# martenlienen/generative-turbulence

Measured on AMD Instinct MI355X. Metric: U-Net fwd+bwd voxels/sec (DDPM training step, 192x64x48x4), higher is better.
Workload: dtype bf16

## Files before the change

### generative-turbulence_amd/csrc/tdx_resize.hip

```cpp
#include "tdx_common.h"
#include <stdlib.h>

struct AxisMap {
    int in, out;
    float scale;
};
__host__ __device__ inline AxisMap make_axis(int in, int out) {
    AxisMap a;
    a.in = in; a.out = out;
    a.scale = out > 1 ? (float)(in - 1) / (float)(out - 1) : 0.0f;
    return a;
}
__host__ __device__ __forceinline__ void axis_taps(const AxisMap& a, int o, int& i0, int& i1, float& w1) {
    const float src = a.scale * (float)o;
    i0 = min((int)src, a.in - 1);
    w1 = fminf(fmaxf(src - (float)i0, 0.0f), 1.0f);
    i1 = i0 + ((i0 + 1 < a.in) ? 1 : 0);
}

struct TileGrid {
    int nx, ny, nz;
    int sy, sz;
    int tx, ty, tz;
};
// ... 192 lines not shown
}
__host__ __device__ __forceinline__ void axis_span(const AxisMap& a, int i, int& first, int& cnt) {
    int lo, hi;
    axis_range(a, i, lo, hi);
    first = hi + 1;
    int last = lo - 1;
    for (int o = lo; o <= hi; ++o)
        if (axis_weight(a, o, i) != 0.f) {
            first = min(first, o);
            last = o;
        }
    cnt = last - first + 1;
    if (cnt < 0) cnt = 0;
}

template <typename T, int K>
__global__ void __launch_bounds__(256)
resize_bwd_kernel(const T* __restrict__ dy, const T* __restrict__ add, T* __restrict__ dx, AxisMap ax, AxisMap ay, AxisMap az,
                  int C, TileGrid tg) {
    __shared__ int s_first[3][RS_MAXT], s_cnt[3][RS_MAXT];
    __shared__ float s_w[3][RS_MAXT][RS_KMAX];
    int b, ix0, iy0, iz0;
    tile_origin(tg, b, ix0, iy0, iz0);
    if (threadIdx.x < 3 * RS_MAXT) {
        const int a = threadIdx.x / RS_MAXT, k = threadIdx.x % RS_MAXT;
        const AxisMap& m = a == 0 ? ax : (a == 1 ? ay : az);
        const int i = min((a == 0 ? ix0 : (a == 1 ? iy0 : iz0)) + k, m.in - 1);
        int f, c;
        axis_span(m, i, f, c);
        s_first[a][k] = f; s_cnt[a][k] = c;
        for (int j = 0; j < RS_KMAX; ++j) s_w[a][k][j] = j < c ? axis_weight(m, f + j, i) : 0.f;
    }
    __syncthreads();
    const int L = C >> 3;
    const int per_pass = 256 / L;
    const int lc = (int)threadIdx.x % L;
    const int nvox = tg.tx * tg.ty * tg.tz;
    if ((int)threadIdx.x >= per_pass * L) return;
    for (int slot = (int)threadIdx.x / L; slot < nvox; slot += per_pass) {
        const int kz = slot & (tg.tz - 1), ky = (slot >> tg.sz) & (tg.ty - 1), kx = slot >> (tg.sz + tg.sy);
        const int ix = ix0 + kx, iy = iy0 + ky, iz = iz0 + kz;
        if (ix >= ax.in || iy >= ay.in || iz >= az.in) continue;
        const int fx = s_first[0][kx], cx = s_cnt[0][kx], fy = s_first[1][ky], cy = s_cnt[1][ky], fz = s_first[2][kz];
        float wz[K];
        int oz[K];
#pragma unroll
        for (int k = 0; k < K; ++k) {
            oz[k] = min(fz + k, az.out - 1);
            wz[k] = s_w[2][kz][k];
        }
        const T* gb = dy + ((int64_t)b * ax.out * ay.out * az.out) * C + lc * 8;
        float acc[8];
#pragma unroll
        for (int j = 0; j < 8; ++j) acc[j] = 0.f;
        for (int a = 0; a < cx; ++a) {
            const float wx = s_w[0][kx][a];
            for (int bb = 0; bb < cy; ++bb) {
                const float wxy = wx * s_w[1][ky][bb];
                const T* row = gb + (((int64_t)(fx + a) * ay.out + (fy + bb)) * az.out) * C;
                Raw8<T> t[K];
#pragma unroll
                for (int k = 0; k < K; ++k) t[k].load(row + (int64_t)oz[k] * C);
                __builtin_amdgcn_sched_barrier(0);
#pragma unroll
                for (int k = 0; k < K; ++k) {
                    const float w = wxy * wz[k];
                    const Vec8<T> v = t[k].get();
#pragma unroll
                    for (int j = 0; j < 8; ++j) acc[j] += w * v.v[j];
                }
            }
        }
        const int64_t di = ((((int64_t)b * ax.in + ix) * ay.in + iy) * az.in + iz) * C + lc * 8;
        if (add != nullptr) {
            Vec8<T> a;
            a.load(add + di);
#pragma unroll
            for (int j = 0; j < 8; ++j) acc[j] += a.v[j];
        }
        Vec8<T> o;
#pragma unroll
        for (int j = 0; j < 8; ++j) o.v[j] = acc[j];
        o.store(dx + di);
    }
}

template <typename T>
__global__ void __launch_bounds__(256)
resize_bwd_generic_kernel(const T* __restrict__ dy, const T* __restrict__ add, T* __restrict__ dx, AxisMap ax, AxisMap ay,
                          AxisMap az, int C, int64_t total) {
    const int L = C >> 3;
    int64_t i = (int64_t)blockIdx.x * blockDim.x + threadIdx.x;
    if (i >= total) return;
    const int lc = (int)(i % L);
    int64_t v = i / L;
    const int iz = (int)(v % az.in); v /= az.in;
    const int iy = (int)(v % ay.in); v /= ay.in;
    const int ix = (int)(v % ax.in);
    const int b = (int)(v / ax.in);
    int x0, x1, y0, y1, z0, z1;
    axis_range(ax, ix, x0, x1);
    axis_range(ay, iy, y0, y1);
    axis_range(az, iz, z0, z1);
    const T* gb = dy + ((int64_t)b * ax.out * ay.out * az.out) * C + lc * 8;
    float acc[8];
#pragma unroll
    for (int j = 0; j < 8; ++j) acc[j] = 0.f;
    for (int ox = x0; ox <= x1; ++ox) {
        const float wx = axis_weight(ax, ox, ix);
        if (wx == 0.f) continue;
        for (int oy = y0; oy <= y1; ++oy) {
            const float wxy = wx * axis_weight(ay, oy, iy);
            if (wxy == 0.f) continue;
            const T* row = gb + (((int64_t)ox * ay.out + oy) * az.out) * C;
            for (int oz = z0; oz <= z1; ++oz) {
                const float w = wxy * axis_weight(az, oz, iz);
                if (w == 0.f) continue;
                Vec8<T> t;
                t.load(row + (int64_t)oz * C);
#pragma unroll
                for (int j = 0; j < 8; ++j) acc[j] += w * t.v[j];
            }
        }
    }
    const int64_t di = ((((int64_t)b * ax.in + ix) * ay.in + iy) * az.in + iz) * C + lc * 8;
    if (add != nullptr) {
        Vec8<T> a;
        a.load(add + di);
#pragma unroll
        for (int j = 0; j < 8; ++j) acc[j] += a.v[j];
    }
    Vec8<T> o;
#pragma unroll
    for (int j = 0; j < 8; ++j) o.v[j] = acc[j];
    o.store(dx + di);
}

static int resize_args_ok(int B, int Xi, int Yi, int Zi, int Xo, int Yo, int Zo, int C) {
    return B > 0 && Xi > 0 && Yi > 0 && Zi > 0 && Xo > 0 && Yo > 0 && Zo > 0 && C > 0;
}
static TileGrid make_tiles(int X, int Y, int Z, int C, int64_t samples = 0) {
    const int L = C >> 3;
    int vox = 256;
    while (vox > 8 && vox * L > 8 * 256) vox >>= 1;
    const int one_pass = 256 / L > 8 ? 256 / L : 8;
    while (samples > 0 && vox > one_pass && samples * X * Y * Z / vox < 1024) vox >>= 1;
    TileGrid t;
    t.tz = 8; t.ty = 8; t.tx = 4;
    while (t.tx * t.ty * t.tz > vox && t.tx > 1) t.tx >>= 1;
    while (t.tx * t.ty * t.tz > vox && t.ty > 1) t.ty >>= 1;
    while (t.tx * t.ty * t.tz > vox && t.tz > 1) t.tz >>= 1;
    t.sy = 0; while ((1 << t.sy) < t.ty) ++t.sy;
    t.sz = 0; while ((1 << t.sz) < t.tz) ++t.sz;
    t.nx = ceil_div(X, t.tx); t.ny = ceil_div(Y, t.ty); t.nz = ceil_div(Z, t.tz);
    return t;
}
extern "C" int tdx_resize_fwd(const void* x, void* y, int B, int Xi, int Yi, int Zi, int Xo, int Yo, int Zo, int C,
                              int dtype, void* stream) {
    TDX_CHECK_ARG(x && y && resize_args_ok(B, Xi, Yi, Zi, Xo, Yo, Zo, C));
    if (C % 8 || C / 8 > 256) return TDX_ESHAPE;
    const TileGrid tg = make_tiles(Xo, Yo, Zo, C, B);
    const int64_t blocks = (int64_t)B * tg.nx * tg.ny * tg.nz;
    const AxisMap mx = make_axis(Xi, Xo), my = make_axis(Yi, Yo), mz = make_axis(Zi, Zo);
    if (C <= 64 && !((tg.tx | tg.ty | tg.tz) & 1) && Xo > Xi && Yo > Yi && Zo > Zi && pair_window_ok(mx) &&
        pair_window_ok(my) && pair_window_ok(mz)) {
        TDX_DISPATCH_DTYPE(dtype, hipLaunchKernelGGL((resize_up_pairs_kernel<T>), dim3((unsigned)blocks), dim3(256), 0,
                                                      as_stream(stream), (const T*)x, (T*)y, mx, my, mz, C, tg));
        return tdx_launch_status();
    }
    TDX_DISPATCH_DTYPE(dtype, hipLaunchKernelGGL((resize_fwd_kernel<T>), dim3((unsigned)blocks), dim3(256), 0,
                                                  as_stream(stream), (const T*)x, (T*)y, make_axis(Xi, Xo),
                                                  make_axis(Yi, Yo), make_axis(Zi, Zo), C, tg));
    return tdx_launch_status();
}

static int axis_max_span(const AxisMap& a) {
    int m = 0;
    for (int i = 0; i < a.in; ++i) {
        int f, c;
        axis_span(a, i, f, c);
        m = c > m ? c : m;
    }
    return m;
}

extern "C" int tdx_resize_bwd(const void* dy, const void* add, void* dx, int B, int Xi, int Yi, int Zi, int Xo, int Yo, int Zo, int C,
                              int dtype, void* stream) {
    TDX_CHECK_ARG(dy && dx && resize_args_ok(B, Xi, Yi, Zi, Xo, Yo, Zo, C));
    if (C % 8 || C / 8 > 256) return TDX_ESHAPE;
    const AxisMap ax = make_axis(Xi, Xo), ay = make_axis(Yi, Yo), az = make_axis(Zi, Zo);
    const int kx = axis_max_span(ax), ky = axis_max_span(ay), kz = axis_max_span(az);
    if (kx > RS_KMAX || ky > RS_KMAX || kz > RS_KMAX) {
        const int64_t total = (int64_t)B * Xi * Yi * Zi * (C / 8);
        TDX_DISPATCH_DTYPE(dtype, hipLaunchKernelGGL((resize_bwd_generic_kernel<T>), dim3(ceil_div(total, 256)), dim3(256), 0,
                                                      as_stream(stream), (const T*)dy, (const T*)add, (T*)dx, ax, ay, az, C, total));
        return tdx_launch_status();
    }
    const TileGrid tg = make_tiles(Xi, Yi, Zi, C, B);
    const dim3 grid((unsigned)((int64_t)B * tg.nx * tg.ny * tg.nz));
#define RS_BWD(KV)                                                                                                     \
    TDX_DISPATCH_DTYPE(dtype, hipLaunchKernelGGL((resize_bwd_kernel<T, KV>), grid, dim3(256), 0, as_stream(stream),     \
                                                  (const T*)dy, (const T*)add, (T*)dx, ax, ay, az, C, tg))
    if (kz <= 2) RS_BWD(2);
    else if (kz <= 4) RS_BWD(4);
    else if (kz <= 6) RS_BWD(6);
    else RS_BWD(RS_KMAX);
#undef RS_BWD
    return tdx_launch_status();
}
```

### generative-turbulence_amd/turbdiff_amd/_lib.py

```python

from __future__ import annotations

import ctypes as C
import os
import threading
from pathlib import Path

import torch

_HERE = Path(__file__).resolve().parent
LIB_PATH = Path(os.environ.get("TDX_LIB", _HERE / "libtdx_hip.so"))

F32, BF16 = 0, 1
F16 = 3
CONV_AUTO, CONV_DIRECT, CONV_MFMA, CONV_SPLIT = 0, 1, 2, 3
F32_SPLIT = 2
WS_CLEAN = 0x100
ACT_NONE, ACT_SILU, ACT_GELU, ACT_RELU, ACT_SOFTPLUS, ACT_TANH = range(6)

_vp, _i, _i64, _u64, _f, _sz = C.c_void_p, C.c_int, C.c_int64, C.c_uint64, C.c_float, C.c_size_t

SIGNATURES = {
    "tdx_version": (_i, []),
    "tdx_arch": (C.c_char_p, []),
    "tdx_switch_count": (_i, []),
    "tdx_switch_name": (C.c_char_p, [_i]),
    "tdx_switch_default": (_i, [_i]),
    "tdx_switch_value": (_i, [_i]),
    "tdx_set_scratch": (_i, [_vp, _sz]),
    "tdx_ncv_to_nvc": (_i, [_vp, _vp, _i, _i, _i64, _i, _i, _vp]),
    "tdx_nvc_to_ncv": (_i, [_vp, _vp, _i, _i, _i64, _i, _i, _vp]),
    "tdx_cast": (_i, [_vp, _vp, _i64, _i, _i, _vp]),
    "tdx_conv3_pack_weight": (_i, [_vp, _vp, _vp, _i, _i, _i, _vp]),
    "tdx_conv3_pack_weights": (_i, [_vp, _i, _i, _vp]),
    "tdx_transpose_many": (_i, [_vp, _i, _vp]),
    "tdx_conv3_fwd": (_i, [_vp, _i, _vp, _i, _vp, _vp, _vp, _i, _i, _i, _i, _i, _i, _i, _vp]),
    "tdx_conv3_uses_ring": (_i, [_i] * 7),
    "tdx_conv3_ring_brick_depth": (_i, [_i] * 7),
    "tdx_conv3_fwd_kernel": (_i, [_i] * 9),
    "tdx_conv3_fwd_gn": (_i, [_vp, _i, _vp, _i, _vp, _vp, _vp, _vp, _i, _f, _vp, _i, _i, _i, _i, _i, _i, _i, _vp]),
    "tdx_conv3_fwd_partial": (_i, [_vp, _i, _i, _vp, _vp, _vp, _i, _vp, _vp, _i, _f, _vp, _i, _i, _i, _i, _i, _i, _i, _vp]),
    "tdx_conv3_bwd_data_workspace_bytes": (_sz, [_i, _i, _i, _i, _i, _i, _i]),
    "tdx_conv3_bwd_data": (_i, [_vp, _vp, _vp, _i, _vp, _i, _i, _i, _i, _i, _i, _i, _i, _i, _vp, _vp]),
    "tdx_conv3_bwd_data_add": (_i, [_vp, _vp, _vp, _i, _vp, _i, _vp, _vp, _i, _i, _i, _i, _i, _i, _i, _vp, _vp]),
    "tdx_conv3_bwd_data_skip_supported": (_i, [_i] * 9),
    "tdx_conv3_bwd_data_skip": (_i, [_vp, _vp, _vp, _i, _vp, _i, _vp, _vp, _i, _i, _i, _i, _i, _i, _i, _vp, _vp]),
    "tdx_conv3_bwd_weight_workspace_bytes": (_sz, [_i, _i, _i]),
    "tdx_conv3_bwd_weight": (_i, [_vp, _i, _vp, _i, _vp, _vp, _vp, _i, _i, _i, _i, _i, _i, _i, _vp, _vp]),
    "tdx_conv3_bwd_weight_plan": (_i, [_i] * 9 + [_vp]),
    "tdx_conv1_fwd": (_i, [_vp, _i, _vp, _i, _vp, _i, _vp, _vp, _vp, _i64, _i, _i, _vp]),
    "tdx_conv1_fwd_gn": (_i, [_vp, _i, _vp, _i, _vp, _i, _vp, _vp, _vp, _vp, _vp, _i, _vp, _i, _i64, _i, _i, _vp]),
    "tdx_conv1_bwd_weight": (_i, [_vp, _i, _vp, _i, _vp, _i, _vp, _i64, _i, _vp]),
    "tdx_conv1_bwd_weight_oc": (_i, [_vp, _i, _vp, _i, _vp, _i, _vp, _i, _i64, _i, _vp]),
    "tdx_encode_fwd": (_i, [_vp, _i, _vp, _vp, _vp, _i, _vp, _vp, _vp, _i, _i64, _i, _i, _vp]),
    "tdx_encode_bwd": (_i, [_vp, _vp, _i, _vp, _i, _vp, _vp, _vp, _vp, _vp, _vp, _i, _i64, _i, _i, _vp]),
    "tdx_decode_fwd": (_i, [_vp, _vp, _vp, _vp, _i, _i64, _i, _i, _i, _vp]),
    "tdx_decode_bwd": (_i, [_vp, _vp, _vp, _vp, _vp, _vp, _i, _i64, _i, _i, _i, _vp]),
    "tdx_gn_workspace_bytes": (_sz, [_i, _i]),
    "tdx_gn_stats": (_i, [_vp, _vp, _i, _i64, _i, _i, _f, _i, _vp, _vp]),
    "tdx_gn_apply": (_i, [_vp, _vp, _vp, _vp, _vp, _vp, _vp, _vp, _i, _i64, _i, _i, _i, _i, _vp]),
    "tdx_gn_apply_decode": (_i, [_vp, _vp, _vp, _vp, _vp, _vp, _vp, _vp, _i, _i64, _i, _i, _i, _i, _vp]),
    "tdx_gn_apply_encoded": (_i, [_vp, _vp, _vp, _vp, _vp, _i, _vp, _vp, _vp, _i, _vp, _vp, _vp, _i, _i64, _i, _i, _i, _vp]),
    "tdx_gn_apply_decode_act": (_i, [_vp, _vp, _vp, _vp, _vp, _vp, _vp, _vp, _i, _i64, _i, _i, _i, _i, _i, _vp]),
    "tdx_gn_apply_encoded_act": (_i, [_vp, _vp, _vp, _vp, _vp, _i, _vp, _vp, _vp, _i, _vp, _vp, _vp, _i, _i64, _i, _i, _i, _i, _vp]),
    "tdx_gn_bwd": (_i, [_vp] * 12 + [_i, _i64, _i, _i, _i, _i, _vp, _vp]),
    "tdx_bn_workspace_bytes": (_sz, [_i64, _i]),
    "tdx_bn_stats": (_i, [_vp, _vp, _vp, _i64, _i, _f, _i, _vp, _vp]),
    "tdx_bn_apply": (_i, [_vp, _vp, _vp, _vp, _vp, _i64, _vp, _i64, _i, _f, _i, _vp]),
    "tdx_bn_bwd": (_i, [_vp] * 8 + [_i64, _i, _f, _i, _i, _vp, _vp]),
    "tdx_flow_decompose_workspace_bytes": (_sz, [_i] * 7),
    "tdx_flow_decompose_fwd": (_i, [_vp] * 6 + [_i] * 8 + [_vp]),
    "tdx_flow_decompose_bwd": (_i, [_vp] * 9 + [_i] * 8 + [_vp, _vp]),
    "tdx_resize_fwd": (_i, [_vp, _vp] + [_i] * 9 + [_vp]),
    "tdx_resize_bwd": (_i, [_vp, _vp, _vp] + [_i] * 9 + [_vp]),
    "tdx_attn_fwd": (_i, [_vp, _vp, _vp, _i, _i, _i, _i, _i, _vp]),
    "tdx_attn_bwd": (_i, [_vp, _vp, _vp, _vp, _vp, _i, _i, _i, _i, _i, _vp, _vp]),
    "tdx_attn_bwd_workspace_bytes": (_sz, [_i, _i, _i, _i]),
    "tdx_cell_mask": (_i, [_vp, _i64, _vp, _i64, _vp]),
    "tdx_q_sample": (_i, [_vp, _vp, _vp, _vp, _vp, _i, _vp, _i, _vp, _i, _i, _i64, _vp]),
    "tdx_p_sample_step": (_i, [_vp] * 7 + [_i, _vp, _i, _i, _vp, _i, _i, _i64, _vp]),
    "tdx_p_sample_step_rng": (_i, [_vp] * 5 + [_i, _vp, _i, _i, _vp, _i, _i, _i64, _u64, _vp, _vp, _vp]),
    "tdx_p_sample_step_lv": (_i, [_vp] * 8 + [_i, _vp, _i, _i, _vp, _i, _i, _i64, _vp]),
    "tdx_p_sample_step_lv_rng": (_i, [_vp] * 6 + [_i, _vp, _i, _i, _vp, _i, _i, _i64, _u64, _vp, _vp, _vp]),
    "tdx_ddim_step": (_i, [_vp] * 7 + [_i, _vp, _vp, _vp, _i, _i, _vp, _i, _i, _i64, _vp]),
    "tdx_ddim_step_rng": (_i, [_vp] * 5 + [_i, _vp, _vp, _vp, _i, _i, _vp, _i, _i, _i64, _u64, _vp, _vp, _vp]),
    "tdx_masked_loss": (_i, [_vp, _vp, _vp, _i64, _i, _vp, _vp, _i, _i, _i64, _vp, _vp]),
    "tdx_masked_loss_dyn": (_i, [_vp, _vp, _vp, _vp, _i, _vp, _vp, _i, _i, _i64, _vp, _vp]),
    "tdx_masked_loss_workspace_bytes": (_sz, []),
    "tdx_elbo_loss": (_i, [_vp] * 5 + [_i64, _vp, _vp, _vp, _i, _i, _i, _i, C.c_double, _vp, _vp, _i, _i, _i64, _vp, _vp]),
    "tdx_elbo_loss_dyn": (_i, [_vp] * 5 + [_vp, _vp, _vp, _vp, _i, _i, _i, _i, C.c_double, _vp, _vp, _i, _i, _i64, _vp, _vp]),
    "tdx_elbo_loss_workspace_bytes": (_sz, []),
    "tdx_grid_embed": (_i, [_vp, _i, _vp, _i, _vp, _i, _vp, _i, _vp, _vp, _vp, _vp, _vp, _vp, _vp, _i, _i64, _i64, _vp]),
    "tdx_grid_select": (_i, [_vp, _vp, _vp, _vp, _vp, _i, _vp, _i, _vp, _i, _vp, _i, _i, _i64, _i64, _vp]),
    "tdx_cell_embed_fwd": (_i, [_vp, _vp, _vp, _i, _i, _i64, _vp]),
    "tdx_cell_embed_bwd_workspace_bytes": (_sz, [_i, _i]),
    "tdx_cell_embed_bwd": (_i, [_vp, _vp, _vp, _i, _i, _i, _i64, _vp, _vp]),
    "tdx_tke_energy": (_i, [_vp, _vp, _i, _i64, _vp]),
    "tdx_tke_sphere": (_i, [_vp, _vp, _vp, _vp, _vp, _i, _i, _i, _i, _i, _i, _vp]),
    "tdx_fd": (_i, [_vp, _vp, _i, _i, _i, _i, _f, _f, _f, _f, _i, _vp]),
    "tdx_ot_features": (_i, [_vp, _vp, _vp, _vp, _vp, _vp, _i, _i64, _i, _i, _i, _f, _f, _f, _vp]),
    "tdx_ot_workspace_bytes": (_sz, [_i, _i]),
    "tdx_ot_auction": (_i, [_vp, _vp, _i64, _vp, _vp, _i, _vp, _i, _i, _i, C.c_double, _i, _i64, _vp, _i, _i, _vp, _vp, _vp]),
    "tdx_moments_update": (_i, [_vp, _i, _i64, _vp, _vp, _i64, _vp]),
    "tdx_field_stats_workspace_bytes": (_sz, [_i64, _i]),
    "tdx_field_stats": (_i, [_vp, _i64, _i, _i, _i, _i, _i, _vp, _vp, _vp]),
    "tdx_w2n_blocks": (_i, [_i64]),
    "tdx_w2n_assign": (_i, [_vp, _vp, _i64, _vp, _vp, _i, _vp, _vp, _vp, _vp]),
    "tdx_w2n_reduce": (_i, [_vp, _i, _i, _vp, _vp]),
    "tdx_lagprod_workspace_bytes": (_sz, [_i, _i64, _i]),
    "tdx_lagprod_update": (_i, [_vp, _i, _i64, _vp, _vp, _i64, _i, _vp, _vp, _i64, _vp, _vp]),
    "tdx_smooth_residual_workspace_bytes": (_sz, [_i64, _i]),
    "tdx_smooth_residual_update": (_i, [_vp, _i, _i64, _vp, _i, _i, _vp, _vp, _i64, _vp, _vp]),
    "tdx_sqdev_workspace_bytes": (_sz, [_i64, _i]),
    "tdx_sqdev_sum": (_i, [_vp, _vp, _i, _i64, _i, _i, _vp, _vp, _vp]),
    "tdx_fma64_probe": (_i, [_vp, _i, _i, _vp]),
    "tdx_randn": (_i, [_vp, _i64, _u64, _u64, _vp, _vp]),
    "tdx_randn_batched": (_i, [_vp, _i, _i64, _u64, _vp, _vp, _vp]),
    "tdx_convg_apply": (_i, [_vp, _vp, _vp, _vp] + [_i] * 16 + [_vp]),
    "tdx_convg_fold_clamp": (_i, [_vp, _vp, _i, _i, _i, _i, _i, _i, _i, _vp]),
    "tdx_convg_bwd_weight": (_i, [_vp, _vp, _vp, _vp] + [_i] * 15 + [_vp]),
    "tdx_convg_apply_fused": (_i, [_vp, _vp, _vp, _vp] + [_i] * 13 + [_vp, _i, _vp]),
    "tdx_convg_fold_fused": (_i, [_vp] * 6 + [_i] * 7 + [_vp]),
    "tdx_film_supported": (_i, [_i, _i]),
    "tdx_film_fwd": (_i, [_vp, _i, _i, _vp, _i, _vp]),
    "tdx_film_bwd_workspace_bytes": (_sz, [_i, _i, _vp, _i]),
    "tdx_film_bwd": (_i, [_vp, _i, _i, _vp, _i, _vp, _vp, _vp]),
    "tdx_opt_chunk_elems": (_i64, []),
    "tdx_grad_norm": (_i, [_vp, _vp, _vp, _i, _f, _vp, _vp, _vp]),
    "tdx_radam_step": (_i, [_vp, _vp, _vp, _i, _vp, _i64, _f, _f, _f, _f, _i, _vp]),
    "tdx_signal_host": (_i, [_vp, _vp, C.c_uint32, _vp]),
    "tdx_stage_scaled": (_i, [_vp, _i, _f, _vp]),
    "tdx_grad_norm_scaled": (_i, [_vp, _vp, _vp, _i, _f, _f, _vp, _vp, _vp]),
    "tdx_radam_step_scaled": (_i, [_vp, _vp, _vp, _i, _vp, _i64, _f, _f, _f, _f, _i, _vp]),
    "tdx_adam_step": (_i, [_vp, _vp, _vp, _i, _vp, _i64] + [C.c_double] * 5 + [_i, _i, _vp]),
    "tdx_adam_step_scaled": (_i, [_vp, _vp, _vp, _i, _vp, _i64] + [C.c_double] * 5 + [_i, _i, _vp]),
}

FILM_MAX_LAYERS = 32


class FilmLayer(C.Structure):
    _fields_ = [("weight", _vp), ("bias", _vp), ("out", _vp), ("channels", _i)]


class PackJob(C.Structure):
    _fields_ = [("w", _vp), ("wf", _vp), ("wb", _vp), ("Cin", _i), ("Cout", _i)]


class TransposeJob(C.Structure):
    _fields_ = [("src", _vp), ("dst", _vp), ("rows", _i), ("cols", _i)]


class StageItem(C.Structure):
    _fields_ = [("src", _vp), ("dst", _vp), ("n", _i64)]


class FilmGrad(C.Structure):
# ... 176 lines not shown
    if not t.is_contiguous():
        raise RuntimeError("tdx kernels need contiguous tensors")
    return t.data_ptr()


_raw_stream = getattr(torch._C, "_cuda_getCurrentRawStream", None)


def stream(device_index=None):
    if _raw_stream is None:
        return torch.cuda.current_stream(device_index).cuda_stream
    return _raw_stream(torch.cuda.current_device() if device_index is None else device_index)


_ERR = {-1: "TDX_EINVAL (bad argument)", -2: "TDX_ESHAPE (unsupported shape)", -3: "TDX_EDTYPE (unsupported dtype)"}


class KernelTimer:

    def __init__(self, names):
        self.names = set(names)
        self.records = []
        self.pending_work = 0.0

    def summary(self, where=None):
        torch.cuda.synchronize()
        out = {}
        for name, s, e, work, meta in self.records:
            if where is not None and not where(meta or {}):
                continue
            d = out.setdefault(name, {"launches": 0, "ms": 0.0, "work": 0.0, "bytes": 0.0})
            d["launches"] += 1
            d["ms"] += s.elapsed_time(e)
            d["work"] += work
            d["bytes"] += (meta or {}).get("bytes", 0.0)
        return out


TIMER: KernelTimer | None = None


def call(name: str, *args, work: float = 0.0, meta=None):
    if name in ARENA_USERS or (name in DET_ARENA_USERS and deterministic()):
        with _LAUNCH_LOCK:
            ensure_scratch()
            rc = _launch(name, args, work, meta)
    else:
        rc = _launch(name, args, work, meta)
    if rc != 0:
        raise RuntimeError(f"{name} failed: {_ERR.get(rc, f'hipError {rc}')}")


def _launch(name, args, work, meta):
    t = TIMER
    if t is not None and name in t.names:
        s, e = torch.cuda.Event(enable_timing=True), torch.cuda.Event(enable_timing=True)
        s.record()
        rc = getattr(load(), name)(*args)
        e.record()
        t.records.append((name, s, e, work, meta() if callable(meta) else meta))
        return rc
    return getattr(load(), name)(*args)


def query(name: str, *args) -> int:
    return int(getattr(load(), name)(*args))


def kernel_sources_fingerprint(pattern: str = "tdx_conv*") -> str | None:
    import hashlib

    src = _HERE.parent / "csrc"
    files = sorted(f for f in src.glob(pattern) if f.suffix in (".hip", ".h"))
    if not files:
        return None
    h = hashlib.sha256()
    for f in files:
        h.update(f.name.encode())
        h.update(f.read_bytes())
    return h.hexdigest()[:16]


KERNEL_DIRECT, KERNEL_BRICK, KERNEL_SMALL, KERNEL_RING = 0, 1, 2, 3


WGRAD_DIRECT, WGRAD_BRICK16, WGRAD_SMALL, WGRAD_RING, WGRAD_BRICK_F32, WGRAD_SPLIT, WGRAD_SPLIT_RING = range(7)
WGRAD_KERNELS = ("direct", "brick16", "small", "ring", "brick_f32", "split", "split_ring")
WGRAD_PLAN_INTS = 16
WGRAD_PLAN_FIELDS = ("kernel", "tile", "depth", "nsplit", "nslab", "sum_unpack", "nbg", "xs", "gx", "ngroups", "max_slabs", "nbricks", "order")


def conv3_bwd_weight_plan(C1, C2, Cout, B, X, Y, Z, dtype: int, impl: int) -> dict:
    buf = (C.c_int * WGRAD_PLAN_INTS)()
    status = int(load().tdx_conv3_bwd_weight_plan(C1, C2, Cout, B, X, Y, Z, dtype, impl, buf))
    plan = {k: int(buf[i]) for i, k in enumerate(WGRAD_PLAN_FIELDS)}
    plan["kernel"] = WGRAD_KERNELS[plan["kernel"]]
    plan["status"] = status
    return plan


def conv3_fwd_meta(C1, C2, Cout, B, X, Y, Z, dt, real=None):
    es = 2 if dt in H16_DTYPES else 4
    cin = real or (C1 + C2)
    return {"kind": query("tdx_conv3_fwd_kernel", C1, C2, Cout, B, X, Y, Z, dtype_code(dt), conv_impl()),
            "bytes": float((cin + Cout) * B * X * Y * Z * es + 27 * cin * Cout * es)}
```

### include/tdx.h

```cpp
#ifndef TDX_H
#define TDX_H

#include <stddef.h>
#include <stdint.h>

#ifdef __cplusplus
extern "C" {
#endif

#define TDX_F32 0
#define TDX_BF16 1

#define TDX_OK 0
#define TDX_EINVAL (-1)
#define TDX_ESHAPE (-2)
#define TDX_EDTYPE (-3)

#define TDX_CONV_AUTO 0
#define TDX_CONV_DIRECT 1
#define TDX_CONV_MFMA 2
#define TDX_CONV_SPLIT 3
#define TDX_F32_SPLIT 2
#define TDX_F16 3
#define TDX_WS_CLEAN 0x100
// ... 70 lines not shown
#define TDX_WGRAD_PLAN_KERNEL 0
#define TDX_WGRAD_PLAN_TILE 1
#define TDX_WGRAD_PLAN_DEPTH 2
#define TDX_WGRAD_PLAN_NSPLIT 3
#define TDX_WGRAD_PLAN_NSLAB 4
#define TDX_WGRAD_PLAN_SUM_UNPACK 5
#define TDX_WGRAD_PLAN_NBG 6
#define TDX_WGRAD_PLAN_XS 7
#define TDX_WGRAD_PLAN_GX 8
#define TDX_WGRAD_PLAN_NGROUPS 9
#define TDX_WGRAD_PLAN_MAX_SLABS 10
#define TDX_WGRAD_PLAN_NBRICKS 11
#define TDX_WGRAD_PLAN_ORDER 12
#define TDX_WGRAD_PLAN_INTS 16
int tdx_conv3_bwd_weight_plan(int C1, int C2, int Cout, int B, int X, int Y, int Z, int dtype, int impl, int* plan);

int tdx_conv1_fwd(const void* x1, int C1, const void* x2, int C2, const float* w, int ldw, const float* bias,
                  const void* add, void* y, int64_t rows, int Cout, int dtype, void* stream);
int tdx_conv1_fwd_gn(const void* x1, int C1, const void* x2, int C2, const float* w, int ldw, const float* bias,
                     const void* h, const float* stats, const float* gamma, const float* beta, int groups, void* y,
                     int B, int64_t V, int Cout, int dtype, void* stream);
int tdx_conv1_bwd_weight(const void* x, int Cin, const void* dy, int Cout, float* dw, int ldw, float* dbias,
                         int64_t rows, int dtype, void* stream);
int tdx_conv1_bwd_weight_oc(const void* x, int Cin, const void* dy, int Cout, float* dw, int ldw, float* dbias,
                            int accumulate, int64_t rows, int dtype, void* stream);

int tdx_encode_fwd(const float* x, int Fx, const float* wx, const float* bx, const float* c, int Fc, const float* wc,
                   const float* bc, void* y, int B, int64_t V, int D, int dtype, void* stream);
int tdx_encode_bwd(const void* dy, const float* x, int Fx, const float* c, int Fc, const float* wc, float* dwx,
                   float* dbx, float* dwc, float* dbc, float* dc, int B, int64_t V, int D, int dtype, void* stream);
int tdx_decode_fwd(const void* h, const float* w, const float* bias, float* y, int B, int64_t V, int D, int F, int dtype,
                   void* stream);
int tdx_decode_bwd(const float* dy, const void* h, const float* w, void* dh, float* dw, float* db, int B, int64_t V, int D,
                   int F, int dtype, void* stream);

size_t tdx_gn_workspace_bytes(int B, int C);
int tdx_gn_stats(const void* x, float* stats, int B, int64_t V, int C, int G, float eps, int dtype, void* workspace,
                 void* stream);
#define TDX_ACT_NONE 0
#define TDX_ACT_SILU 1
#define TDX_ACT_GELU 2
#define TDX_ACT_RELU 3
#define TDX_ACT_SOFTPLUS 4
#define TDX_ACT_TANH 5
int tdx_gn_apply(const void* x, const float* stats, const float* gamma, const float* beta, const float* scale,
                 const float* shift, const void* res, void* y, int B, int64_t V, int C, int G, int act, int dtype,
                 void* stream);
int tdx_gn_apply_encoded(const void* x, const float* stats, const float* gamma, const float* beta, const float* x_raw, int Fx,
                         const float* wx, const float* bx, const float* c_raw, int Fc, const float* wc, const float* bc,
                         void* y, int B, int64_t V, int D, int G, int dtype, void* stream);
int tdx_gn_apply_encoded_act(const void* x, const float* stats, const float* gamma, const float* beta, const float* x_raw,
                             int Fx, const float* wx, const float* bx, const float* c_raw, int Fc, const float* wc,
                             const float* bc, void* y, int B, int64_t V, int D, int G, int dtype, int act, void* stream);
int tdx_gn_apply_decode(const void* x, const float* stats, const float* gamma, const float* beta, const void* res,
                        const float* w, const float* bias, float* out, int B, int64_t V, int C, int G, int F, int dtype,
                        void* stream);
int tdx_gn_apply_decode_act(const void* x, const float* stats, const float* gamma, const float* beta, const void* res,
                            const float* w, const float* bias, float* out, int B, int64_t V, int C, int G, int F, int dtype,
                            int act, void* stream);
int tdx_gn_bwd(const void* x, const void* dy, const float* stats, const float* gamma, const float* beta,
               const float* scale, const float* shift, void* dx, float* dgamma, float* dbeta, float* dscale,
               float* dshift, int B, int64_t V, int C, int G, int act, int dtype, void* workspace, void* stream);

size_t tdx_bn_workspace_bytes(int64_t rows, int C);
int tdx_bn_stats(const void* x, float* stats, float* var, int64_t rows, int C, float eps, int dtype, void* workspace,
                 void* stream);
int tdx_bn_apply(const void* x, const float* stats, const float* gamma, const float* beta, const void* add, int64_t add_rows,
                 void* y, int64_t rows, int C, float slope, int dtype, void* stream);
int tdx_bn_bwd(const void* x, const void* dy, const float* stats, const float* gamma, const float* beta, void* dx,
               float* dgamma, float* dbeta, int64_t rows, int C, float slope, int training, int dtype, void* workspace,
               void* stream);

size_t tdx_flow_decompose_workspace_bytes(int B, int T, int L, int F, int X, int Y, int Z);
int tdx_flow_decompose_fwd(const float* xx, const float* spatial_w, const float* temporal_w, void* bar, void* tilde, void* prime,
                           int B, int T, int L, int F, int X, int Y, int Z, int dtype, void* stream);
int tdx_flow_decompose_bwd(const float* xx, const float* spatial_w, const float* temporal_w, const void* gbar, const void* gtilde,
                           const void* gprime, float* gxx, float* gspatial, float* gtemporal, int B, int T, int L, int F, int X,
                           int Y, int Z, int dtype, void* workspace, void* stream);

int tdx_resize_fwd(const void* x, void* y, int B, int Xi, int Yi, int Zi, int Xo, int Yo, int Zo, int C, int dtype,
                   void* stream);
int tdx_resize_bwd(const void* dy, const void* add, void* dx, int B, int Xi, int Yi, int Zi, int Xo, int Yo, int Zo, int C,
                   int dtype, void* stream);

int tdx_attn_fwd(const void* qkv, void* out, float* lse, int B, int N, int H, int D, int dtype, void* stream);
int tdx_attn_bwd(const void* qkv, const void* out, const float* lse, const void* dout, void* dqkv, int B, int N, int H,
                 int D, int dtype, void* workspace, void* stream);
size_t tdx_attn_bwd_workspace_bytes(int B, int N, int H, int D);


int tdx_cell_mask(const int64_t* cell_idx, int64_t n_cells, uint8_t* mask, int64_t V, void* stream);

int tdx_q_sample(const float* x0, const float* noise, const float* sqrt_ac, const float* sqrt_1mac, const int64_t* t,
                 int t_stride, const uint8_t* mask, int keep_bcs, float* out, int B, int F, int64_t V, void* stream);

int tdx_p_sample_step(const float* x_t, const float* eps, const float* z, const float* z2, const float* x_bcs,
                      const uint8_t* mask, const float* sched, int T, const int64_t* t, int noise_bcs, int clip,
                      float* out, int B, int F, int64_t V, void* stream);

int tdx_p_sample_step_rng(const float* x_t, const float* eps, const float* x_bcs, const uint8_t* mask, const float* sched,
                          int T, int64_t* t, int noise_bcs, int clip, float* out, int B, int F, int64_t V, uint64_t seed,
                          const uint64_t* stream_ids, uint64_t* offset_dev, void* stream);

int tdx_p_sample_step_lv(const float* x_t, const float* model_out, const float* z, const float* z2, const float* x_bcs,
                         const uint8_t* mask, const float* sched, const float* posterior_log_var, int T, const int64_t* t,
                         int noise_bcs, int clip, float* out, int B, int F, int64_t V, void* stream);

int tdx_p_sample_step_lv_rng(const float* x_t, const float* model_out, const float* x_bcs, const uint8_t* mask,
                             const float* sched, const float* posterior_log_var, int T, int64_t* t, int noise_bcs, int clip,
                             float* out, int B, int F, int64_t V, uint64_t seed, const uint64_t* stream_ids,
                             uint64_t* offset_dev, void* stream);

int tdx_ddim_step(const float* x_t, const float* eps, const float* z, const float* z2, const float* x_bcs,
                  const uint8_t* mask, const float* tab, int S, const int64_t* k, const int64_t* tau, const int64_t* t,
                  int noise_bcs, int clip, float* out, int B, int F, int64_t V, void* stream);

int tdx_ddim_step_rng(const float* x_t, const float* eps, const float* x_bcs, const uint8_t* mask, const float* tab, int S,
                      int64_t* k, const int64_t* tau, int64_t* t, int noise_bcs, int clip, float* out, int B, int F,
                      int64_t V, uint64_t seed, const uint64_t* stream_ids, uint64_t* offset_dev, void* stream);

int tdx_masked_loss(const float* eps_hat, const float* noise, const uint8_t* mask, int64_t n_cells, int l1,
                    float* loss, float* grad, int B, int F, int64_t V, void* workspace, void* stream);
int tdx_masked_loss_dyn(const float* eps_hat, const float* noise, const unsigned char* mask, const int64_t* n_cells_dev,
                        int l1, float* loss, float* grad, int B, int F, int64_t V, void* workspace, void* stream);
size_t tdx_masked_loss_workspace_bytes(void);

int tdx_elbo_loss(const float* out, const float* noise, const float* x_start, const float* x_t, const uint8_t* mask,
                  int64_t n_cells, const int64_t* t, const float* sched, const float* posterior_log_var, int T, int l1,
                  int clip, int detach_mean, double elbo_weight, float* loss, float* grad, int B, int F, int64_t V,
                  void* workspace, void* stream);
int tdx_elbo_loss_dyn(const float* out, const float* noise, const float* x_start, const float* x_t, const uint8_t* mask,
                      const int64_t* n_cells_dev, const int64_t* t, const float* sched, const float* posterior_log_var,
                      int T, int l1, int clip, int detach_mean, double elbo_weight, float* loss, float* grad, int B, int F,
                      int64_t V, void* workspace, void* stream);
size_t tdx_elbo_loss_workspace_bytes(void);

int tdx_grid_embed(const float* s0, int d0, const float* s1, int d1, const float* s2, int d2, const float* s3, int d3,
                   const int32_t* cell_of, const int32_t* ovr_of, const float* ovr_val, const uint32_t* ovr_mask,
                   const float* shift, const float* scale, float* x, int B, int64_t n_cells, int64_t V, void* stream);
int tdx_grid_select(const float* x, const int64_t* cell_idx, const float* mean, const float* std, float* o0, int d0,
                    float* o1, int d1, float* o2, int d2, float* o3, int d3, int B, int64_t n_cells, int64_t V,
                    void* stream);
int tdx_cell_embed_fwd(const uint8_t* types, const float* table, float* out, int n_types, int D, int64_t V, void* stream);
size_t tdx_cell_embed_bwd_workspace_bytes(int n_types, int D);
int tdx_cell_embed_bwd(const uint8_t* types, const float* dC, float* dtable, int accumulate, int n_types, int D, int64_t V,
                       void* workspace, void* stream);

int tdx_tke_energy(const float* u, float* tke, int B, int64_t V, void* stream);
int tdx_tke_sphere(const float* fft, const float* p, const float* w, const float* k, float* E, int B, int X, int Y, int Z,
                   int N, int K, void* stream);

#define TDX_FD_CURL 0
#define TDX_FD_DIVERGENCE 1
#define TDX_FD_ENSTROPHY 2
int tdx_fd(const float* u, float* out, int B, int X, int Y, int Z, float two_hx, float two_hy, float two_hz, float dv,
           int mode, void* stream);
int tdx_ot_features(const float* u_grid, const float* u_cells, const float* p_cells, const int64_t* unpadded_idx,
                    const float* scale, float* out, int S, int64_t n_cells, int X, int Y, int Z, float two_hx, float two_hy,
                    float two_hz, void* stream);

#define TDX_OT_OK 0
#define TDX_OT_ROUND_CAP 1
#define TDX_OT_BID_CAP 2
#define TDX_OT_BAD_JOB 3
#define TDX_OT_NONFINITE 4
size_t tdx_ot_workspace_bytes(int max_n, int slots);
// ... 116 lines not shown
```

Before: 172.2 million.

## Add paired-output resize backward kernel that shares upsampled gradient windows

Adds a trilinear-resize backward kernel for upsampling, where each thread computes a 2x2x2 group of input-gradient voxels. The group reads one shared window of output gradients, so overlapping taps are loaded once instead of once per input voxel. Per-axis weight windows are precomputed in shared memory, loads are software-pipelined across rows, and tile sizes adapt to keep enough workgroups busy. It adds routing logic and a query entry point, at the cost of more registers and a 2-block launch bound.

```diff
diff --git a/generative-turbulence_amd/csrc/tdx_resize.hip b/generative-turbulence_amd/csrc/tdx_resize.hip
--- a/generative-turbulence_amd/csrc/tdx_resize.hip
+++ b/generative-turbulence_amd/csrc/tdx_resize.hip
@@ -298,6 +298,191 @@
 #pragma unroll
         for (int j = 0; j < 8; ++j) o.v[j] = acc[j];
         o.store(dx + di);
+    }
+}
+
+#define RS_PW 7
+struct PairWin {
+    int base, n;
+    float w[2][RS_PW];
+};
+__host__ __device__ __forceinline__ bool pair_win(const AxisMap& a, int i_even, PairWin& p) {
+    int lo = a.out, hi = -1;
+#pragma unroll
+    for (int q = 0; q < 2; ++q) {
+        int f, c;
+        if (i_even + q >= a.in) continue;
+        axis_span(a, i_even + q, f, c);
+        if (c > 0) {
+            lo = min(lo, f);
+            hi = max(hi, f + c - 1);
+        }
+    }
+    if (hi < lo) lo = hi = 0;
+    const bool ok = hi - lo + 1 <= RS_PW;
+    p.base = lo;
+    p.n = min(hi - lo + 1, RS_PW);
+#pragma unroll
+    for (int q = 0; q < 2; ++q)
+#pragma unroll
+        for (int s = 0; s < RS_PW; ++s) p.w[q][s] = (s < p.n && i_even + q < a.in) ? axis_weight(a, lo + s, i_even + q) : 0.f;
+    return ok;
+}
+static int bwd_pair_window(const AxisMap& a) {
+    if (a.out <= a.in) return 0;
+    PairWin p;
+    int m = 0;
+    for (int i = 0; i < a.in; i += 2) {
+        if (!pair_win(a, i, p)) return 0;
+        m = p.n > m ? p.n : m;
+    }
+    return m;
+}
+
+struct PairTiles {
+    int nx, ny, nz;
+    int px, py, pz;
+    int sy, sz;
+};
+
+template <typename T, int KZ>
+__global__ void __launch_bounds__(256, 2)
+resize_bwd_pairs_kernel(const T* __restrict__ dy, const T* __restrict__ add, T* __restrict__ dx, AxisMap ax, AxisMap ay,
+                        AxisMap az, int C, PairTiles pt) {
+    __shared__ PairWin s_p[3][RS_MAXT];
+    int t = blockIdx.x;
+    const int iz0 = (t % pt.nz) * pt.pz * 2; t /= pt.nz;
+    const int iy0 = (t % pt.ny) * pt.py * 2; t /= pt.ny;
+    const int ix0 = (t % pt.nx) * pt.px * 2;
+    const int b = t / pt.nx;
+    if (threadIdx.x < 3 * RS_MAXT) {
+        const int a = threadIdx.x / RS_MAXT, k = threadIdx.x % RS_MAXT;
+        const AxisMap& m = a == 0 ? ax : (a == 1 ? ay : az);
+        PairWin p;
+        pair_win(m, min((a == 0 ? ix0 : (a == 1 ? iy0 : iz0)) + 2 * k, (m.in - 1) & ~1), p);
+        s_p[a][k] = p;
+    }
+    __syncthreads();
+    const int L = C >> 3;
+    const int lc = (int)threadIdx.x % L, slot = (int)threadIdx.x / L;
+    if (slot >= pt.px * pt.py * pt.pz) return;
+    const int kz = slot & (pt.pz - 1), ky = (slot >> pt.sz) & (pt.py - 1), kx = slot >> (pt.sz + pt.sy);
+    const int ix = ix0 + 2 * kx, iy = iy0 + 2 * ky, iz = iz0 + 2 * kz;
+    if (ix >= ax.in || iy >= ay.in || iz >= az.in) return;
+    const PairWin& wx = s_p[0][kx];
+    const PairWin& wy = s_p[1][ky];
+    const PairWin& wz = s_p[2][kz];
+    const int bx = wx.base, nx = wx.n, by = wy.base, ny = wy.n, bz = wz.base;
+    const char* gb = reinterpret_cast<const char*>(dy + ((int64_t)b * ax.out * ay.out * az.out) * C);
+    const unsigned row_bytes = (unsigned)(az.out * C) * (unsigned)sizeof(T);
+    unsigned oz[KZ];
+#pragma unroll
+    for (int k = 0; k < KZ; ++k) oz[k] = (unsigned)(min(bz + k, az.out - 1) * C + lc * 8) * (unsigned)sizeof(T);
+    typedef float f2 __attribute__((ext_vector_type(2)));
+    f2 acc[2][2][2][4];
+#pragma unroll
+    for (int i = 0; i < 32; ++i) (&acc[0][0][0][0])[i] = (f2)(0.f);
+    f2 py[2][2][4];
+#pragma unroll
+    for (int i = 0; i < 16; ++i) (&py[0][0][0])[i] = (f2)(0.f);
+    constexpr int NB = sizeof(T) == 4 ? 1 : (KZ <= 6 ? 3 : 2);
+    Raw8<T> r[NB][KZ];
+    const unsigned plane_step = (unsigned)(ay.out - ny + 1) * row_bytes;
+    unsigned irow = (unsigned)(bx * ay.out + by) * row_bytes;
+    int isx = 0, isy = 0;
+    auto issue = [&](Raw8<T>* q) {
+#pragma unroll
+        for (int k = 0; k < KZ; ++k) q[k].load(reinterpret_cast<const T*>(gb + (irow + oz[k])));
+        if (isy + 1 < ny) {
+            ++isy;
+            irow += row_bytes;
+        } else if (isx + 1 < nx) {
+            ++isx;
+            isy = 0;
+            irow += plane_step;
+        }
+    };
+    int csx = 0, csy = 0;
+    auto reduce = [&](const Raw8<T>* q) {
+        const bool live = csx < nx;
+        const float wy0 = live ? wy.w[0][csy] : 0.f, wy1 = live ? wy.w[1][csy] : 0.f;
+        f2 p0[4], p1[4];
+#pragma unroll
+        for (int j = 0; j < 4; ++j) p0[j] = p1[j] = (f2)(0.f);
+#pragma unroll
+        for (int k = 0; k < KZ; ++k) {
+            const Vec8<T> v = q[k].get();
+            const float w0 = wz.w[0][k], w1 = wz.w[1][k];
+#pragma unroll
+            for (int j = 0; j < 4; ++j) {
+                const f2 vv = {v.v[2 * j], v.v[2 * j + 1]};
+                p0[j] += w0 * vv;
+                p1[j] += w1 * vv;
+            }
+        }
+#pragma unroll
+        for (int j = 0; j < 4; ++j) {
+            py[0][0][j] += wy0 * p0[j];
+            py[0][1][j] += wy0 * p1[j];
+            py[1][0][j] += wy1 * p0[j];
+            py[1][1][j] += wy1 * p1[j];
+        }
+        if (csy + 1 < ny) {
+            ++csy;
+        } else {
+            if (live) {
+                const float wx0 = wx.w[0][csx], wx1 = wx.w[1][csx];
+#pragma unroll
+                for (int i = 0; i < 16; ++i) {
+                    (&acc[0][0][0][0])[i] += wx0 * (&py[0][0][0])[i];
+                    (&acc[1][0][0][0])[i] += wx1 * (&py[0][0][0])[i];
+                    (&py[0][0][0])[i] = (f2)(0.f);
+                }
+            }
+            csy = 0;
+            ++csx;
+        }
+    };
+#pragma unroll
+    for (int s = 0; s + 1 < NB; ++s) issue(r[s]);
+    const int nrows = nx * ny;
+    int done = 0;
+#pragma unroll 1
+    do {
+#pragma unroll
+        for (int s = 0; s < NB; ++s) {
+            issue(r[(s + NB - 1) % NB]);
+            __builtin_amdgcn_sched_barrier(0);
+            reduce(r[s]);
+        }
+        done += NB;
+    } while (done < nrows);
+    const int64_t d0 = ((((int64_t)b * ax.in + ix) * ay.in + iy) * az.in + iz) * C + lc * 8;
+    const int64_t sx1 = (int64_t)ay.in * az.in * C, sy1 = (int64_t)az.in * C;
+    const bool inx = ix + 1 < ax.in, iny = iy + 1 < ay.in, inz = iz + 1 < az.in;
+    Raw8<T> ad[2][2][2];
+    if (add != nullptr) {
+#pragma unroll
+        for (int q = 0; q < 8; ++q) {
+            const int qx = q >> 2, qy = (q >> 1) & 1, qz = q & 1;
+            const bool in = (!qx || inx) && (!qy || iny) && (!qz || inz);
+            ad[qx][qy][qz].load(add + d0 + (in ? qx * sx1 + qy * sy1 + qz * C : 0));
+        }
+    }
+#pragma unroll
+    for (int q = 0; q < 8; ++q) {
+        const int qx = q >> 2, qy = (q >> 1) & 1, qz = q & 1;
+        if ((qx && !inx) || (qy && !iny) || (qz && !inz)) continue;
+        Vec8<T> o;
+        if (add != nullptr) {
+            const Vec8<T> a = ad[qx][qy][qz].get();
+#pragma unroll
+            for (int j = 0; j < 8; ++j) o.v[j] = acc[qx][qy][qz][j >> 1][j & 1] + a.v[j];
+        } else {
+#pragma unroll
+            for (int j = 0; j < 8; ++j) o.v[j] = acc[qx][qy][qz][j >> 1][j & 1];
+        }
+        o.store(dx + d0 + qx * sx1 + qy * sy1 + qz * C);
     }
 }
 
@@ -400,13 +585,75 @@
     return m;
 }
 
+static int pair_tile_fit(int n, int cap) {
+    for (int p = cap; p > 1; p >>= 1)
+        if ((ceil_div(n, p) * p - n) * 8 <= n) return p;
+    return 1;
+}
+#ifndef RS_BWD_PAIRS_MIN_WGS
+#define RS_BWD_PAIRS_MIN_WGS 1024
+#endif
+static PairTiles make_pair_tiles(int B, int X, int Y, int Z, int C, int& threads) {
+    const int L = C >> 3;
+    const int bx = ceil_div(X, 2), by = ceil_div(Y, 2), bz = ceil_div(Z, 2);
+    PairTiles t;
+    for (threads = 256;; threads >>= 1) {
+        int blk = 1;
+        while (blk * 2 * L <= threads) blk <<= 1;
+        t.pz = pair_tile_fit(bz, blk < RS_MAXT ? blk : RS_MAXT);
+        t.py = pair_tile_fit(by, blk / t.pz < RS_MAXT ? blk / t.pz : RS_MAXT);
+        t.px = blk / (t.pz * t.py) < RS_MAXT ? blk / (t.pz * t.py) : RS_MAXT;
+        t.nx = ceil_div(bx, t.px); t.ny = ceil_div(by, t.py); t.nz = ceil_div(bz, t.pz);
+        if (threads == 64 || threads / 2 < L || (int64_t)B * t.nx * t.ny * t.nz >= RS_BWD_PAIRS_MIN_WGS) break;
+    }
+    t.sy = 0; while ((1 << t.sy) < t.py) ++t.sy;
+    t.sz = 0; while ((1 << t.sz) < t.pz) ++t.sz;
+    return t;
+}
+
+#define RS_BWD_PAIRS_MAXC 128
+static int resize_bwd_route(const AxisMap& ax, const AxisMap& ay, const AxisMap& az, int C, int& kwin) {
+    kwin = 0;
+    if (C <= RS_BWD_PAIRS_MAXC && (int64_t)ax.out * ay.out * az.out * C <= ((int64_t)1 << 29)) {
+        const int wx = bwd_pair_window(ax), wy = wx ? bwd_pair_window(ay) : 0, wz = wy ? bwd_pair_window(az) : 0;
+        if (wz) {
+            kwin = wz <= 6 ? 6 : RS_PW;
+            return TDX_RESIZE_BWD_PAIRS;
+        }
+    }
+    const int kx = axis_max_span(ax), ky = axis_max_span(ay), kz = axis_max_span(az);
+    if (kx > RS_KMAX || ky > RS_KMAX || kz > RS_KMAX) return TDX_RESIZE_BWD_GENERIC;
+    return kz <= 2 ? 2 : (kz <= 4 ? 4 : (kz <= 6 ? 6 : RS_KMAX));
+}
+
+extern "C" int tdx_resize_bwd_kernel(int B, int Xi, int Yi, int Zi, int Xo, int Yo, int Zo, int C) {
+    TDX_CHECK_ARG(resize_args_ok(B, Xi, Yi, Zi, Xo, Yo, Zo, C));
+    if (C % 8 || C / 8 > 256) return TDX_ESHAPE;
+    int kwin;
+    return resize_bwd_route(make_axis(Xi, Xo), make_axis(Yi, Yo), make_axis(Zi, Zo), C, kwin);
+}
+
 extern "C" int tdx_resize_bwd(const void* dy, const void* add, void* dx, int B, int Xi, int Yi, int Zi, int Xo, int Yo, int Zo, int C,
                               int dtype, void* stream) {
     TDX_CHECK_ARG(dy && dx && resize_args_ok(B, Xi, Yi, Zi, Xo, Yo, Zo, C));
     if (C % 8 || C / 8 > 256) return TDX_ESHAPE;
     const AxisMap ax = make_axis(Xi, Xo), ay = make_axis(Yi, Yo), az = make_axis(Zi, Zo);
-    const int kx = axis_max_span(ax), ky = axis_max_span(ay), kz = axis_max_span(az);
-    if (kx > RS_KMAX || ky > RS_KMAX || kz > RS_KMAX) {
+    int kwin;
+    const int route = resize_bwd_route(ax, ay, az, C, kwin);
+    if (route == TDX_RESIZE_BWD_PAIRS) {
+        int threads;
+        const PairTiles pt = make_pair_tiles(B, Xi, Yi, Zi, C, threads);
+        const dim3 grid((unsigned)((int64_t)B * pt.nx * pt.ny * pt.nz));
+#define RS_BWD_PAIRS(KV)                                                                                                     \
+    TDX_DISPATCH_DTYPE(dtype, hipLaunchKernelGGL((resize_bwd_pairs_kernel<T, KV>), grid, dim3(threads), 0, as_stream(stream), \
+                                                  (const T*)dy, (const T*)add, (T*)dx, ax, ay, az, C, pt))
+        if (kwin == 6) RS_BWD_PAIRS(6);
+        else RS_BWD_PAIRS(RS_PW);
+#undef RS_BWD_PAIRS
+        return tdx_launch_status();
+    }
+    const int kz = route;
+    if (route == TDX_RESIZE_BWD_GENERIC) {
         const int64_t total = (int64_t)B * Xi * Yi * Zi * (C / 8);
         TDX_DISPATCH_DTYPE(dtype, hipLaunchKernelGGL((resize_bwd_generic_kernel<T>), dim3(ceil_div(total, 256)), dim3(256), 0,
                                                       as_stream(stream), (const T*)dy, (const T*)add, (T*)dx, ax, ay, az, C, total));
diff --git a/generative-turbulence_amd/turbdiff_amd/_lib.py b/generative-turbulence_amd/turbdiff_amd/_lib.py
--- a/generative-turbulence_amd/turbdiff_amd/_lib.py
+++ b/generative-turbulence_amd/turbdiff_amd/_lib.py
@@ -73,6 +73,7 @@
     "tdx_flow_decompose_bwd": (_i, [_vp] * 9 + [_i] * 8 + [_vp, _vp]),
     "tdx_resize_fwd": (_i, [_vp, _vp] + [_i] * 9 + [_vp]),
     "tdx_resize_bwd": (_i, [_vp, _vp, _vp] + [_i] * 9 + [_vp]),
+    "tdx_resize_bwd_kernel": (_i, [_i] * 8),
     "tdx_attn_fwd": (_i, [_vp, _vp, _vp, _i, _i, _i, _i, _i, _vp]),
     "tdx_attn_bwd": (_i, [_vp, _vp, _vp, _vp, _vp, _i, _i, _i, _i, _i, _vp, _vp]),
     "tdx_attn_bwd_workspace_bytes": (_sz, [_i, _i, _i, _i]),
@@ -415,6 +416,7 @@
 
 
 KERNEL_DIRECT, KERNEL_BRICK, KERNEL_SMALL, KERNEL_RING = 0, 1, 2, 3
+RESIZE_BWD_GENERIC, RESIZE_BWD_PAIRS = 0, 1
 
 
 WGRAD_DIRECT, WGRAD_BRICK16, WGRAD_SMALL, WGRAD_RING, WGRAD_BRICK_F32, WGRAD_SPLIT, WGRAD_SPLIT_RING = range(7)
diff --git a/include/tdx.h b/include/tdx.h
--- a/include/tdx.h
+++ b/include/tdx.h
@@ -176,6 +176,9 @@
                    void* stream);
 int tdx_resize_bwd(const void* dy, const void* add, void* dx, int B, int Xi, int Yi, int Zi, int Xo, int Yo, int Zo, int C,
                    int dtype, void* stream);
+#define TDX_RESIZE_BWD_GENERIC 0
+#define TDX_RESIZE_BWD_PAIRS 1
+int tdx_resize_bwd_kernel(int B, int Xi, int Yi, int Zi, int Xo, int Yo, int Zo, int C);
 
 int tdx_attn_fwd(const void* qkv, void* out, float* lse, int B, int N, int H, int D, int dtype, void* stream);
 int tdx_attn_bwd(const void* qkv, const void* out, const float* lse, const void* dout, void* dqkv, int B, int N, int H,
```

Result: no change. 171.2 million (-0.6%).
